# owensgroup/sparsify.me

Measured on AMD Instinct MI355X. Metric: effective GF/s (2:4 spmma vs dense gemm) on ResNet-50 layer shapes, higher is better.
Workload: dtype f16

## Files before the change

include/sparsifyme.h:

```cpp
#ifndef SPARSIFYME_H_
#define SPARSIFYME_H_

#include <stddef.h>
#include <stdint.h>

#ifdef __cplusplus
extern "C" {
#endif

#define SM_STATUS_SUCCESS 0
#define SM_STATUS_INVALID_VALUE 1
#define SM_STATUS_NOT_SUPPORTED 2
#define SM_STATUS_LAUNCH_FAILED 3
#define SM_STATUS_NO_DEVICE 4

#define SM_PRUNE_TILE 0
#define SM_PRUNE_STRIP 1

#define SM_OP_N 0
#define SM_OP_T 1

typedef void* sm_stream_t;

const char* sm_version(void);
// ... 78 lines not shown
int sm_prune24_spmma_f16(const void* A_in, void* A_out, const void* B, void* C, size_t m, size_t n, size_t k, size_t lda,
                         size_t batch, size_t strideA, size_t strideB, size_t strideC, int alg, int* d_valid, float alpha,
                         float beta, sm_stream_t stream);
int sm_prune24_spmma_bf16(const void* A_in, void* A_out, const void* B, void* C, size_t m, size_t n, size_t k, size_t lda,
                          size_t batch, size_t strideA, size_t strideB, size_t strideC, int alg, int* d_valid, float alpha,
                          float beta, sm_stream_t stream);

int sm_spmma_f16(const void* blob, const void* B, void* C, size_t m, size_t n, size_t k,
                 size_t batch, size_t strideB, size_t strideC, float alpha, float beta,
                 sm_stream_t stream);
int sm_spmma_f32(const void* blob, const float* B, float* C, size_t m, size_t n, size_t k,
                 size_t batch, size_t strideB, size_t strideC, float alpha, float beta,
                 sm_stream_t stream);

int sm_spmma_fused_f16(const void* A, const void* B, void* C, size_t m, size_t n, size_t k, size_t lda,
                       size_t batch, size_t strideA, size_t strideB, size_t strideC, float alpha,
                       float beta, sm_stream_t stream);

int sm_spmma_f16_grouped(size_t count, const void* const* blobs, const void* const* B, void* const* C, size_t m, size_t n, size_t k,
                         size_t batch, size_t strideB, size_t strideC, float alpha, float beta, sm_stream_t stream);
int sm_spmma_bf16_grouped(size_t count, const void* const* blobs, const void* const* B, void* const* C, size_t m, size_t n, size_t k,
                          size_t batch, size_t strideB, size_t strideC, float alpha, float beta, sm_stream_t stream);

int sm_spmma_fused_f16_grouped(size_t count, const void* const* A, const void* const* B, void* const* C, size_t m, size_t n,
                               size_t k, size_t lda, size_t batch, size_t strideA, size_t strideB, size_t strideC,
                               float alpha, float beta, sm_stream_t stream);
int sm_spmma_fused_bf16_grouped(size_t count, const void* const* A, const void* const* B, void* const* C, size_t m, size_t n,
                                size_t k, size_t lda, size_t batch, size_t strideA, size_t strideB, size_t strideC,
                                float alpha, float beta, sm_stream_t stream);

int sm_spmma_fused_workspace_size(size_t* bytes);
int sm_spmma_fused_workspace_state(const void* workspace, int* state, sm_stream_t stream);
int sm_spmma_fused_streamk_plan(size_t rows, size_t n, size_t k, size_t problems, int* takes, unsigned* plan);
#define SM_FUSED_FORM_NOT_TAKEN 0
#define SM_FUSED_FORM_EMPTY 1
#define SM_FUSED_FORM_THIN 2
#define SM_FUSED_FORM_SPAN 3
#define SM_FUSED_FORM_STREAMK 4
#define SM_FUSED_FORM_BIG 5
#define SM_FUSED_FORM_DIRECT64 6
#define SM_FUSED_FORM_DIRECT128 7
#define SM_FUSED_FORM_DIRECT128_NT 8
#define SM_FUSED_FORM_ASTAT 9
#define SM_FUSED_FORM_WIDEP 10
#define SM_FUSED_FORM_WIDE 11
#define SM_FUSED_FORM_WIDE_NT 12
#define SM_FUSED_FLAG_A_ALIGNED 1u
#define SM_FUSED_FLAG_B_ALIGNED 2u
#define SM_FUSED_FLAG_C_ALIGNED 4u
#define SM_FUSED_FLAG_WORKSPACE 8u
#define SM_FUSED_FLAG_EPILOGUE 16u
int sm_spmma_fused_form(size_t m, size_t n, size_t k, size_t lda, size_t batch, size_t count, size_t strideA, size_t strideB, size_t strideC,
                        float beta, unsigned flags, size_t cus, int* form);
int sm_gemm_rowmajor_f16_ws(const void* A, const void* B, void* C, size_t m, size_t n, size_t k, size_t lda, size_t batch, size_t strideA,
                            size_t strideB, size_t strideC, float alpha, float beta, void* workspace, size_t workspace_bytes, sm_stream_t stream);
int sm_gemm_rowmajor_bf16_ws(const void* A, const void* B, void* C, size_t m, size_t n, size_t k, size_t lda, size_t batch, size_t strideA,
                             size_t strideB, size_t strideC, float alpha, float beta, void* workspace, size_t workspace_bytes, sm_stream_t stream);
int sm_gemm_batched_f16_ws(const void* const* A_ptrs, const void* const* B_ptrs, void* const* C_ptrs, size_t m, size_t n, size_t k, size_t batch,
                           int transpose_a, int transpose_b, float alpha, float beta, void* workspace, size_t workspace_bytes, sm_stream_t stream);
int sm_spmma_fused_f16_ws(const void* A, const void* B, void* C, size_t m, size_t n, size_t k, size_t lda, size_t batch, size_t strideA,
                          size_t strideB, size_t strideC, float alpha, float beta, void* workspace, size_t workspace_bytes, sm_stream_t stream);
int sm_spmma_fused_bf16_ws(const void* A, const void* B, void* C, size_t m, size_t n, size_t k, size_t lda, size_t batch, size_t strideA,
                           size_t strideB, size_t strideC, float alpha, float beta, void* workspace, size_t workspace_bytes, sm_stream_t stream);
int sm_spmma_fused_f16_grouped_ws(size_t count, const void* const* A, const void* const* B, void* const* C, size_t m, size_t n,
                                  size_t k, size_t lda, size_t batch, size_t strideA, size_t strideB, size_t strideC,
                                  float alpha, float beta, void* workspace, size_t workspace_bytes, sm_stream_t stream);
int sm_spmma_fused_bf16_grouped_ws(size_t count, const void* const* A, const void* const* B, void* const* C, size_t m, size_t n,
                                   size_t k, size_t lda, size_t batch, size_t strideA, size_t strideB, size_t strideC,
                                   float alpha, float beta, void* workspace, size_t workspace_bytes, sm_stream_t stream);

#define SM_BIAS_COL 0
#define SM_BIAS_ROW 1
#define SM_ACT_NONE 0
#define SM_ACT_RELU 1
#define SM_ACT_CLIPPED_RELU 2
#define SM_ACT_LEAKY_RELU 3
#define SM_ACT_HARDSWISH 4
typedef struct {
  const float* bias;
  int bias_dim;
  int act;
  float act_arg;
  const void* R;
  size_t strideR;
} sm_epilogue_t;
int sm_spmma_f16_ex(const void* blob, const void* B, void* D, size_t m, size_t n, size_t k, size_t batch, size_t strideB,
                    size_t strideD, float alpha, float beta, const sm_epilogue_t* epilogue, sm_stream_t stream);
int sm_spmma_bf16_ex(const void* blob, const void* B, void* D, size_t m, size_t n, size_t k, size_t batch, size_t strideB,
                     size_t strideD, float alpha, float beta, const sm_epilogue_t* epilogue, sm_stream_t stream);
int sm_spmma_fused_f16_ex(const void* A, const void* B, void* D, size_t m, size_t n, size_t k, size_t lda, size_t batch,
                          size_t strideA, size_t strideB, size_t strideD, float alpha, float beta, const sm_epilogue_t* epilogue,
                          sm_stream_t stream);
int sm_spmma_fused_bf16_ex(const void* A, const void* B, void* D, size_t m, size_t n, size_t k, size_t lda, size_t batch,
                           size_t strideA, size_t strideB, size_t strideD, float alpha, float beta, const sm_epilogue_t* epilogue,
                           sm_stream_t stream);

int sm_linear24_f16(const void* blob, const void* X, void* Y, size_t tokens, size_t out_features, size_t in_features, size_t ldx,
                    size_t ldy, float alpha, float beta, const sm_epilogue_t* epilogue, sm_stream_t stream);
int sm_linear24_bf16(const void* blob, const void* X, void* Y, size_t tokens, size_t out_features, size_t in_features, size_t ldx,
                     size_t ldy, float alpha, float beta, const sm_epilogue_t* epilogue, sm_stream_t stream);

int sm_linear24_fp8(const void* blob, const void* X, void* Y, size_t tokens, size_t out_features, size_t in_features, size_t ldx,
                    size_t ldy, int fmt_w, int fmt_x, int out_type, float alpha, float beta, const float* w_scale, const float* x_scale,
                    const sm_epilogue_t* epilogue, sm_stream_t stream);
#define SM_LINEAR24_FORM_NOT_TAKEN 0
#define SM_LINEAR24_FORM_EMPTY 1
// ... 305 lines not shown
```

sparsify.me_amd/__init__.py:

```python
import ctypes
import os
import subprocess

_HERE = os.path.dirname(os.path.abspath(__file__))
LIB_PATH = os.environ.get("SPARSIFYME_LIB") or os.path.join(_HERE, "libsparsifyme.so")

PRUNE_TILE = 0
PRUNE_STRIP = 1
STATUS_SUCCESS, STATUS_INVALID_VALUE, STATUS_NOT_SUPPORTED, STATUS_LAUNCH_FAILED, STATUS_NO_DEVICE = 0, 1, 2, 3, 4

_lib = None

_c_size = ctypes.c_size_t
_c_ptr = ctypes.c_void_p
_c_f = ctypes.c_float
_c_i = ctypes.c_int

_SIGS = {
    "sm_device_check": [],
    "sm_sparsify_positional": [_c_ptr, _c_ptr, _c_size, _c_size, _c_size, _c_size, _c_size, _c_f, _c_ptr],
    "sm_sparsify_positional_f16": [_c_ptr, _c_ptr, _c_size, _c_size, _c_f, _c_ptr],
    "sm_sparsify_positional_f32": [_c_ptr, _c_ptr, _c_size, _c_size, _c_f, _c_ptr],
    "sm_sparsify_positional_f64": [_c_ptr, _c_ptr, _c_size, _c_size, _c_f, _c_ptr],
    "sm_prune24_f16": [_c_ptr, _c_ptr, _c_size, _c_size, _c_size, _c_i, _c_ptr],
# ... 43 lines not shown
                            _c_ptr],
    "sm_spmm_bell_batched_workspace_size": [_c_size, _c_size, _c_size, ctypes.POINTER(_c_size)],
    "sm_spmm_bell_batched_f32": [_c_ptr, _c_ptr, _c_size, _c_size, _c_size, _c_size, _c_ptr, _c_ptr, _c_size, _c_size, _c_f,
                                 _c_f, _c_ptr, _c_ptr],
    "sm_spmm_coo_workspace_size": [_c_size, ctypes.POINTER(_c_size)],
    "sm_spmm_coo_packed_workspace_size": [_c_size, _c_size, ctypes.POINTER(_c_size)],
    "sm_spmm_coo_f32_packed": [_c_size, _c_size, _c_size, _c_size, _c_size, _c_ptr, _c_ptr, _c_ptr, _c_ptr, _c_ptr, _c_f, _c_f,
                               _c_ptr, _c_size, _c_ptr],
    "sm_spmm_coo_f32_ws": [_c_size, _c_size, _c_size, _c_size, _c_size, _c_ptr, _c_ptr, _c_ptr, _c_ptr, _c_ptr, _c_f, _c_f,
                           _c_ptr, _c_ptr],
    "sm_spmm_coo_fast_workspace_size": [_c_size, _c_size, _c_size, _c_size, ctypes.POINTER(_c_size)],
    "sm_spmm_coo_fast_flag": [_c_ptr, ctypes.POINTER(_c_i), _c_ptr],
    "sm_spmm_coo_fast_form": [_c_size, _c_size, _c_size, _c_size, _c_size, _c_f],
    "sm_spmm_coo_f32_fast": [_c_size, _c_size, _c_size, _c_size, _c_size, _c_ptr, _c_ptr, _c_ptr, _c_ptr, _c_ptr, _c_f, _c_f,
                             _c_ptr, _c_size, _c_ptr],
    "sm_fill_uniform_f16": [_c_ptr, _c_size, ctypes.c_uint64, _c_f, _c_f, _c_ptr],
    "sm_fill_uniform_f32": [_c_ptr, _c_size, ctypes.c_uint64, _c_f, _c_f, _c_ptr],
    "sm_copy_bytes": [_c_ptr, _c_ptr, _c_size, _c_ptr],
}
_SIGS["sm_prune24_compress24_f16"] = [_c_ptr, _c_ptr, _c_size, _c_size, _c_size, _c_size, _c_size, _c_ptr, _c_ptr, _c_i, _c_ptr]
_SIGS["sm_prune24_compress24_bf16"] = _SIGS["sm_prune24_compress24_f16"]
_SIGS["sm_prune24_spmma_f16"] = [_c_ptr, _c_ptr, _c_ptr, _c_ptr] + [_c_size] * 8 + [_c_i, _c_ptr, _c_f, _c_f, _c_ptr]
_SIGS["sm_prune24_spmma_bf16"] = _SIGS["sm_prune24_spmma_f16"]
_SIGS["sm_prune24_compress24_f32"] = _SIGS["sm_prune24_compress24_f16"]
_SIGS["sm_prune24_form"] = [_c_ptr, _c_ptr, _c_size, _c_size, _c_size, _c_size, _c_i, ctypes.POINTER(_c_i), ctypes.POINTER(ctypes.c_uint)]
_SIGS["sm_prune24_check_form"] = [_c_ptr, _c_ptr, _c_size, _c_size, _c_size, _c_size, ctypes.POINTER(_c_i)]
_SIGS["sm_compress24_form"] = [_c_ptr, _c_ptr, _c_size, _c_size, _c_size, _c_size, _c_size, _c_size, ctypes.POINTER(_c_i)]
_SIGS["sm_decompress24_form"] = _SIGS["sm_compress24_form"]
_SIGS["sm_prune24_compress24_form"] = [_c_ptr, _c_ptr, _c_size, _c_size, _c_size, _c_size, _c_size, _c_ptr, _c_size, _c_i, _c_size,
                                       ctypes.POINTER(_c_i), ctypes.POINTER(ctypes.c_uint)]
_SIGS["sm_conv_spmma_fused_f16"] = [_c_ptr, _c_ptr, _c_ptr] + [_c_size] * 10 + [_c_f, _c_f, _c_ptr]
_SIGS["sm_conv_spmma_fused_bf16"] = _SIGS["sm_conv_spmma_fused_f16"]
_SIGS["sm_conv_spmma_fused_plan"] = [_c_size] * 10 + [ctypes.c_uint, ctypes.POINTER(_c_i), ctypes.POINTER(ctypes.c_uint)]
_SIGS["sm_transpose"] = [_c_ptr, _c_ptr] + [_c_size] * 8 + [_c_ptr]
_SIGS["sm_conv_out_size"] = [_c_size, _c_size, _c_size, _c_size, _c_size, ctypes.POINTER(_c_size)]
_SIGS["sm_im2col_f16"] = [_c_ptr] + [_c_size] * 9 + [_c_ptr, _c_ptr]
_SIGS["sm_im2col_compress24_f16"] = [_c_ptr] + [_c_size] * 9 + [_c_ptr, _c_ptr]
for _name in ("sm_prune24", "sm_prune24_check", "sm_compress24", "sm_decompress24"):
    _SIGS[_name + "_i8"] = _SIGS[_name + "_f16"]
_SIGS["sm_spmma_fused_i8"] = [_c_ptr, _c_ptr, _c_ptr] + [_c_size] * 8 + [_c_i, _c_ptr]
_SIGS["sm_spmma_fused_i8_q"] = [_c_ptr, _c_ptr, _c_ptr] + [_c_size] * 8 + [_c_f, _c_ptr]
_SIGS["sm_transpose_i8"] = [_c_ptr, _c_ptr, _c_size, _c_size, _c_ptr]
_SIGS["sm_spmma_i8"] = [_c_ptr, _c_ptr, _c_ptr, _c_size, _c_size, _c_size, _c_size, _c_size, _c_size, _c_i, _c_ptr]
_SIGS["sm_spmma_i8_q"] = [_c_ptr, _c_ptr, _c_ptr, _c_size, _c_size, _c_size, _c_size, _c_size, _c_size, _c_f, _c_ptr]
for _name in ("sm_prune24", "sm_prune24_check", "sm_compress24", "sm_decompress24", "sm_spmma", "sm_spmma_fused",
              "sm_gemm_rowmajor", "sm_fill_uniform", "sm_im2col", "sm_im2col_compress24"):
    _SIGS[_name + "_bf16"] = _SIGS[_name + "_f16"]
_SIGS["sm_spmma_fused_f32_split_prepare"] = [_c_ptr, _c_size, _c_size, _c_size, _c_size, _c_i, _c_ptr, _c_size, _c_ptr]
_SIGS["sm_spmma_fused_f32_split_prepared"] = [_c_ptr, _c_ptr, _c_ptr] + [_c_size] * 8 + [_c_i, _c_size, _c_f, _c_f, _c_ptr]
_SIGS["sm_spmma_fused_workspace_size"] = [ctypes.POINTER(_c_size)]
_SIGS["sm_spmma_fused_workspace_state"] = [_c_ptr, ctypes.POINTER(_c_i), _c_ptr]
_SIGS["sm_spmma_fused_streamk_plan"] = [_c_size, _c_size, _c_size, _c_size, ctypes.POINTER(_c_i), ctypes.POINTER(ctypes.c_uint)]
_SIGS["sm_spmma_fused_form"] = [_c_size] * 9 + [_c_f, ctypes.c_uint, _c_size, ctypes.POINTER(_c_i)]
_SIGS["sm_gemm_rowmajor_f16_ws"] = [_c_ptr, _c_ptr, _c_ptr] + [_c_size] * 8 + [_c_f, _c_f, _c_ptr, _c_size, _c_ptr]
_SIGS["sm_gemm_rowmajor_bf16_ws"] = _SIGS["sm_gemm_rowmajor_f16_ws"]
_SIGS["sm_gemm_batched_f16_ws"] = [_c_ptr, _c_ptr, _c_ptr, _c_size, _c_size, _c_size, _c_size, _c_i, _c_i, _c_f, _c_f, _c_ptr, _c_size, _c_ptr]
_SIGS["sm_spmma_fused_f16_ws"] = [_c_ptr, _c_ptr, _c_ptr] + [_c_size] * 8 + [_c_f, _c_f, _c_ptr, _c_size, _c_ptr]
_SIGS["sm_spmma_fused_bf16_ws"] = _SIGS["sm_spmma_fused_f16_ws"]
_SIGS["sm_spmma_fused_f16_grouped_ws"] = [_c_size, _c_ptr, _c_ptr, _c_ptr] + [_c_size] * 8 + [_c_f, _c_f, _c_ptr, _c_size, _c_ptr]
_SIGS["sm_spmma_fused_bf16_grouped_ws"] = _SIGS["sm_spmma_fused_f16_grouped_ws"]
_SIGS["sm_spmm_bell_f16"] = _SIGS["sm_spmm_bell_f32"]
_SIGS["sm_spmm_bell_bf16"] = _SIGS["sm_spmm_bell_f32"]
_SIGS["sm_spmm_bell_batched_f16"] = [_c_ptr, _c_ptr, _c_size, _c_size, _c_size, _c_size, _c_ptr, _c_ptr, _c_size, _c_size, _c_f, _c_f, _c_ptr]
_SIGS["sm_spmm_bell_batched_bf16"] = _SIGS["sm_spmm_bell_batched_f16"]
_SIGS["sm_prune24_fp8"] = [_c_ptr, _c_ptr, _c_size, _c_size, _c_size, _c_i, _c_i, _c_ptr]
_SIGS["sm_prune24_check_fp8"] = _SIGS["sm_prune24_check_f16"]
_SIGS["sm_compress24_fp8"] = [_c_ptr, _c_size, _c_size, _c_size, _c_size, _c_size, _c_ptr, _c_i, _c_ptr]
_SIGS["sm_decompress24_fp8"] = _SIGS["sm_decompress24_f16"]
_SIGS["sm_spmma_fp8"] = [_c_ptr, _c_ptr, _c_ptr] + [_c_size] * 6 + [_c_i, _c_i, _c_i, _c_f, _c_f, _c_ptr, _c_ptr]
_SIGS["sm_spmma_fused_fp8"] = [_c_ptr, _c_ptr, _c_ptr] + [_c_size] * 8 + [_c_i, _c_i, _c_i, _c_f, _c_f, _c_ptr, _c_ptr]
_SIGS["sm_gemm_rowmajor_fp8"] = _SIGS["sm_spmma_fused_fp8"]
_SIGS["sm_gemm_rowmajor_i8"] = _SIGS["sm_spmma_fused_i8"]
_SIGS["sm_gemm_rowmajor_i8_q"] = _SIGS["sm_spmma_fused_i8_q"]
for _sfx16 in ("f16", "bf16"):
    _SIGS["sm_quantize_rows_fp8_" + _sfx16] = [_c_ptr, _c_size, _c_size, _c_size, _c_ptr, _c_size, _c_ptr, _c_i, _c_ptr]
    _SIGS["sm_quantize_compress24_fp8_" + _sfx16] = [_c_ptr, _c_size, _c_size, _c_size, _c_ptr, _c_ptr, _c_i, _c_ptr]
    _SIGS["sm_quantize_transpose_fp8_" + _sfx16] = [_c_ptr, _c_size, _c_size, _c_size, _c_f, _c_ptr, _c_i, _c_ptr]
for _sfx16 in ("f16", "bf16"):
    _SIGS["sm_spmma_%s_ex" % _sfx16] = _SIGS["sm_spmma_f16"][:-1] + [_c_ptr, _c_ptr]
    _SIGS["sm_spmma_fused_%s_ex" % _sfx16] = _SIGS["sm_spmma_fused_f16"][:-1] + [_c_ptr, _c_ptr]
for _sfx16 in ("f16", "bf16"):
    _SIGS["sm_linear24_" + _sfx16] = [_c_ptr, _c_ptr, _c_ptr] + [_c_size] * 5 + [_c_f, _c_f, _c_ptr, _c_ptr]
_SIGS["sm_linear24_fp8"] = [_c_ptr, _c_ptr, _c_ptr] + [_c_size] * 5 + [_c_i, _c_i, _c_i, _c_f, _c_f, _c_ptr, _c_ptr, _c_ptr, _c_ptr]
_SIGS["sm_linear24_fp8_form"] = [_c_size] * 4 + [ctypes.POINTER(_c_i)]
for _sfx16 in ("f16", "bf16"):
    _SIGS["sm_linear24_glu_" + _sfx16] = [_c_ptr, _c_ptr, _c_ptr] + [_c_size] * 5 + [_c_i, _c_ptr, _c_ptr]
_SIGS["sm_linear24_glu_fp8"] = [_c_ptr, _c_ptr, _c_ptr] + [_c_size] * 5 + [_c_i, _c_i, _c_i, _c_i, _c_ptr, _c_ptr, _c_ptr, _c_ptr]
_SIGS["sm_linear24_glu_form"] = [_c_size] * 4 + [ctypes.POINTER(_c_i)]
for _sfx16 in ("f16", "bf16", "fp8"):
    _SIGS["sm_linear24_grouped_" + _sfx16] = _SIGS["sm_linear24_" + _sfx16][:3] + [_c_ptr, _c_size] + _SIGS["sm_linear24_" + _sfx16][3:]
    _SIGS["sm_linear24_grouped_glu_" + _sfx16] = _SIGS["sm_linear24_glu_" + _sfx16][:3] + [_c_ptr, _c_size] + _SIGS["sm_linear24_glu_" + _sfx16][3:]
_SIGS["sm_linear24_grouped_form"] = [_c_size] * 5 + [ctypes.POINTER(_c_i)]
for _sfx16 in ("f16", "bf16", "fp8"):
    for _g in ("sm_linear24_grouped_", "sm_linear24_grouped_glu_"):
        _SIGS[_g + "gather_" + _sfx16] = _SIGS[_g + _sfx16][:4] + [_c_ptr, _c_size] + _SIGS[_g + _sfx16][4:]
_SIGS["sm_moe_route_workspace_size"] = [_c_size] * 3 + [ctypes.POINTER(_c_size)]
_SIGS["sm_moe_route"] = [_c_ptr] + [_c_size] * 3 + [_c_ptr] * 5 + [_c_size, _c_ptr]
_SIGS["sm_moe_route_form"] = [_c_size] * 3 + [ctypes.POINTER(_c_i)]
for _sfx16 in ("f16", "bf16"):
    _SIGS["sm_moe_combine_" + _sfx16] = [_c_ptr] * 5 + [_c_size] * 6 + [_c_ptr]
_SIGS["sm_moe_combine_form"] = [_c_ptr] * 3 + [_c_size] * 3 + [ctypes.POINTER(_c_i)]
for _sfx3 in ("f16", "bf16", "f32"):
    _SIGS["sm_moe_gate_" + _sfx3] = [_c_ptr] * 4 + [_c_size] * 4 + [_c_i, _c_i, _c_f, _c_ptr]
_SIGS["sm_moe_gate_form"] = [_c_size] * 3 + [ctypes.POINTER(_c_i)]
for _sfx16 in ("f16", "bf16"):
    _SIGS["sm_rmsnorm_" + _sfx16] = [_c_ptr] * 7 + [_c_size] * 6 + [_c_f, _c_i, _c_ptr]
# ... 698 lines not shown


def gemm_rowmajor_i8(A, B, C, m, n, k, lda=None, batch=1, strideA=None, strideB=0, strideC=None, accumulate=False):
    lda = k if lda is None else lda
    strideA = m * lda if strideA is None else strideA
    strideC = m * n if strideC is None else strideC
    if C.dtype != _t().int32:
        raise SparsifymeError("gemm_rowmajor_i8 writes int32; use gemm_rowmajor_i8_q for a requantised int8 result")
    _check(lib().sm_gemm_rowmajor_i8(_dev(A), _dev(B), _dev(C), m, n, k, lda, batch, strideA, strideB, strideC, 1 if accumulate else 0,
                                     _stream()), "sm_gemm_rowmajor_i8")


def gemm_rowmajor_i8_q(A, B, C, m, n, k, scale, lda=None, batch=1, strideA=None, strideB=0, strideC=None):
    lda = k if lda is None else lda
    strideA = m * lda if strideA is None else strideA
    strideC = m * n if strideC is None else strideC
    if C.dtype != _t().int8:
        raise SparsifymeError("gemm_rowmajor_i8_q writes int8")
    _check(lib().sm_gemm_rowmajor_i8_q(_dev(A), _dev(B), _dev(C), m, n, k, lda, batch, strideA, strideB, strideC, float(scale), _stream()),
           "sm_gemm_rowmajor_i8_q")


def spmma_fused_workspace_size():
    out = _c_size(0)
    _check(lib().sm_spmma_fused_workspace_size(ctypes.byref(out)), "sm_spmma_fused_workspace_size")
    return out.value


def spmma_fused_streamk_plan(rows, n, k, problems=1):
    takes = _c_i(0)
    buf = (ctypes.c_uint * 32)()
    _check(lib().sm_spmma_fused_streamk_plan(rows, n, k, problems, ctypes.byref(takes), buf), "sm_spmma_fused_streamk_plan")
    v = list(buf)
    return bool(takes.value), dict(tg=v[0], wg=v[1], groups_full=v[2], tgl=v[3], wgl=v[4], slots=v[5], units=v[6], cut=v[7:16], cutl=v[16:25])


FUSED_FORMS = ("not_taken", "empty", "thin", "span", "streamk", "big", "direct64", "direct128", "direct128_nt", "astat", "widep", "wide", "wide_nt")
FUSED_FLAG_A_ALIGNED, FUSED_FLAG_B_ALIGNED, FUSED_FLAG_C_ALIGNED, FUSED_FLAG_WORKSPACE, FUSED_FLAG_EPILOGUE = 1, 2, 4, 8, 16


def spmma_fused_form(m, n, k, lda=None, batch=1, count=1, strideA=None, strideB=0, strideC=None, beta=0.0, a_aligned=True, b_aligned=True,
                     c_aligned=True, workspace=False, epilogue=False, cus=0):
    lda = k if lda is None else lda
    strideA = m * lda if strideA is None else strideA
    strideC = m * n if strideC is None else strideC
    flags = ((FUSED_FLAG_A_ALIGNED if a_aligned else 0) | (FUSED_FLAG_B_ALIGNED if b_aligned else 0) | (FUSED_FLAG_C_ALIGNED if c_aligned else 0) |
             (FUSED_FLAG_WORKSPACE if workspace else 0) | (FUSED_FLAG_EPILOGUE if epilogue else 0))
    form = _c_i(-1)
    _check(lib().sm_spmma_fused_form(m, n, k, lda, batch, count, strideA, strideB, strideC, float(beta), flags, cus, ctypes.byref(form)),
           "sm_spmma_fused_form")
    return FUSED_FORMS[form.value]


def streamk_whole_panels(plan, panels, nkt):
    cuts = set()
    for g in range(plan["groups_full"]):
        cuts.update(g * plan["tg"] * nkt + c for c in plan["cut"][:plan["wg"] + 1])
    base = plan["groups_full"] * plan["tg"] * nkt
    cuts.update(base + c for c in plan["cutl"][:plan["wgl"] + 1])
    return [t for t in range(panels) if not any(t * nkt < u < (t + 1) * nkt for u in cuts)]


def spmma_fused_workspace_state(ws):
    st = _c_i(-1)
    _check(lib().sm_spmma_fused_workspace_state(_dev(ws), ctypes.byref(st), _stream()), "sm_spmma_fused_workspace_state")
    return st.value


def spmma_fused_workspace():
    return _t().zeros(spmma_fused_workspace_size(), dtype=_t().uint8, device="cuda")


def spmma_fused(A, B, C, m, n, k, lda=None, batch=1, strideA=None, strideB=0, strideC=None, alpha=1.0, beta=0.0, workspace=None,
                epilogue=None):
    lda = k if lda is None else lda
    strideA = m * lda if strideA is None else strideA
    strideC = m * n if strideC is None else strideC
    if epilogue is not None:
        if workspace is not None:
            raise SparsifymeError("spmma_fused: the workspace (stream-K) form takes no epilogue")
        st = epilogue.struct_for(C, strideC, float(beta))
        fn = getattr(lib(), "sm_spmma_fused_%s_ex" % _sfx(A))
        _check(fn(_dev(A), _dev(B), _dev(C), m, n, k, lda, batch, strideA, strideB, strideC, float(alpha), float(beta), ctypes.addressof(st),
                  _stream()), "sm_spmma_fused_ex")
        return
    if workspace is not None:
        fn = getattr(lib(), "sm_spmma_fused_%s_ws" % _sfx(A))
        _check(fn(_dev(A), _dev(B), _dev(C), m, n, k, lda, batch, strideA, strideB, strideC, float(alpha), float(beta), _dev(workspace),
                  workspace.numel() * workspace.element_size(), _stream()), "sm_spmma_fused_ws")
        return
    fn = getattr(lib(), "sm_spmma_fused_" + _sfx(A))
    _check(fn(_dev(A), _dev(B), _dev(C), m, n, k, lda, batch, strideA, strideB, strideC, float(alpha), float(beta), _stream()),
           "sm_spmma_fused")


def spmma_grouped(blobs, Bs, Cs, m, n, k, batch=1, strideB=0, strideC=None, alpha=1.0, beta=0.0):
    if not (len(blobs) == len(Bs) == len(Cs)):
        raise SparsifymeError("spmma_grouped: operand lists differ in length")
    if not blobs:
        return
    if strideC is None:
        strideC = m * n
    fn = getattr(lib(), "sm_spmma_%s_grouped" % _sfx(Bs[0]))
    _check(fn(len(blobs), _ptr_table(blobs), _ptr_table(Bs), _ptr_table(Cs), m, n, k, batch, strideB, strideC, float(alpha), float(beta),
              _stream()), "sm_spmma_grouped")

# ... 190 lines not shown
```

sparsify.me_amd/csrc/spmma_f16_fused.hip:

```cpp
#include "select24.h"
#include "spmma_args.h"

namespace sm {

constexpr int MAXG = 8;
struct FusedArgs {
  const half_t* A[MAXG];
  const half_t* B[MAXG];
  half_t* C[MAXG];
  size_t sA, sB, sC;
  int Mrows, N, K, lda;
  int batch, tiles_m, tiles_n;
  int ngroup;
  float alpha, beta;
  const half_t* const* dAp;
  const half_t* const* dBp;
  half_t* const* dCp;
};

struct FusedArgsEpi : FusedArgs {
  EpiArgs e;
};
template <bool EPI> struct FusedArgsSel { typedef FusedArgs type; };
template <> struct FusedArgsSel<true> { typedef FusedArgsEpi type; };
// ... 482 lines not shown
  const SkPlan pl = sk_plan(panels, nkt, tn, cus);
  const size_t nwg = (size_t)pl.slots * tn;
  if (pl.slots == 0 || nwg > cus || nwg > 1023) return "sm_spmma_fused_*_ws: the shape has more column tiles than the stream-K form has compute units for";
  return nullptr;
}

template <int BN, bool BF = false, bool ANT = true, bool DENSE = false>
static int launch_fused_sk(const FusedArgs& a0, void* workspace, size_t workspace_bytes, hipStream_t st) {
  constexpr int BM = 256;
  static_assert(BN == 256, "sk_launch_limits counts 256-column tiles");
  FusedArgs a = a0;
  a.tiles_m = (a.Mrows + BM - 1) / BM;
  a.tiles_n = (a.N + BN - 1) / BN;
  const size_t panels = (size_t)a.tiles_m * a.batch * a.ngroup;
  if (panels == 0) return SM_STATUS_SUCCESS;
  const size_t nkt = (size_t)a.K / 64;
  const int cus = device_cu_count();
  if (const char* why = sk_launch_limits(panels, (size_t)a.N, (size_t)a.K, (size_t)a.lda, (size_t)cus)) {
    set_error("%s", why);
    return SM_STATUS_NOT_SUPPORTED;
  }
  SkPlan pl = sk_plan(panels, nkt, (size_t)a.tiles_n, (size_t)cus);
  const size_t nwg = (size_t)pl.slots * a.tiles_n;
  if (!workspace || !aligned16(workspace) || workspace_bytes < sk_workspace_bytes(nwg, BN)) {
    set_error("sm_spmma_fused_*_ws: the stream-K form needs a 16-byte aligned workspace of sm_spmma_fused_workspace_size bytes");
    return SM_STATUS_INVALID_VALUE;
  }
  SkArgs s = {};
  s.flags = reinterpret_cast<unsigned*>(workspace);
  s.part = reinterpret_cast<float*>(reinterpret_cast<char*>(workspace) + 4096);
  s.panels = (unsigned)panels; s.slots = pl.slots; s.tg = pl.tg; s.wg = pl.wg; s.groups_full = pl.groups_full; s.tgl = pl.tgl; s.wgl = pl.wgl;
  for (int i = 0; i < 9; ++i) { s.cut[i] = pl.cut[i]; s.cutl[i] = pl.cutl[i]; }
  constexpr size_t lds_main = (size_t)3 * BM * 128 + (size_t)2 * 64 * BN * 2;
  constexpr size_t lds_epi = (size_t)BM * (BN * 2 + 16);
  constexpr size_t lds = lds_main > lds_epi ? lds_main : lds_epi;
  static_assert(lds > 64 * 1024 && lds <= 160 * 1024, "LDS budget of the stream-K kernel (always opted in)");
  return launch_grid<&spmma_f16_fused_sk_kernel<BN, BF, ANT, DENSE>>(nwg, 512, lds, lds, st, "sm_spmma_fused_f16", "spmma_f16_fused_sk_kernel", a, s);
}

static bool sk_takes(size_t rows, size_t problems, size_t n, size_t k, bool astat_shape, size_t cus, SkPlan& pl) {
  if (n <= 128 || k < 128 || k % 64 != 0) return false;
  const size_t nkt = k / 64;
  const size_t panels = (rows + 255) / 256 * problems, tn = (n + 255) / 256;
  const size_t t_big = panels * tn, t_wide = (rows + 127) / 128 * tn * problems;
  pl = sk_plan(panels, nkt, tn, cus);
  if (!pl.slots) return false;
  const double c_sk = (double)pl.units + (pl.wg > 1 ? 8.0 : 0.0);
  const double c_big = (double)((t_big + cus - 1) / cus * nkt), c_wide = 0.6 * (double)((t_wide + cus - 1) / cus * nkt);
  const double c_now = c_big < c_wide ? c_big : c_wide;
  return !astat_shape && pl.wg > 1 && c_sk < 0.85 * c_now;
}

__device__ __attribute__((aligned(256))) const unsigned char sm_fused_zero_page[256] = {0};

template <int BN, bool BF = false, bool DENSE = false, bool EPI = false>
__global__ __launch_bounds__(256) void spmma_f16_fused_span_kernel(const typename FusedArgsSel<EPI>::type p, const unsigned span_lds ,
                                                                   const size_t a_bytes ) {
  constexpr int BM = 128, NW = 4, TM = BM / NW, FM = TM / 16, FN = BN / 16;
  constexpr int SB = 64 * BN * 2;
  extern __shared__ __attribute__((aligned(16))) char smem[];
  const unsigned tid = threadIdx.x, lane = tid & 63u;
  const unsigned wave = __builtin_amdgcn_readfirstlane(tid >> 6);
  const unsigned tiles = (unsigned)p.tiles_m * (unsigned)p.tiles_n;
  const unsigned lid = xcd_remap(blockIdx.x, gridDim.x);
  const unsigned grp = lid / tiles, trem = lid - grp * tiles;
  const unsigned tile_m = trem / (unsigned)p.tiles_n, tile_n = trem - tile_m * (unsigned)p.tiles_n;
  const int m0 = (int)tile_m * BM, n0 = (int)tile_n * BN;
  const int nkt = (p.K + 63) / 64;
  const char* A = reinterpret_cast<const char*>(p.dAp ? p.dAp[grp] : p.A[grp]);
  const half_t* B = p.dBp ? p.dBp[grp] : p.B[grp];
  half_t* C = p.dCp ? p.dCp[grp] : p.C[grp];
  const unsigned rowbytes = (unsigned)p.K * 2u;
  const int rows = p.Mrows - m0 < BM ? p.Mrows - m0 : BM;
  EpiBias<FM, FN> eb;
  if constexpr (EPI) eb = epi_bias_prefetch<FM, FN>(p.e, true, wave * TM, 0, m0, n0, p.Mrows, p.N, lane);

  {
    const size_t s0 = (size_t)m0 * rowbytes;
    const unsigned len = (unsigned)rows * rowbytes;
    const unsigned np = (len + 1023u) / 1024u;
    const size_t last16 = a_bytes - 16;
    for (unsigned pc = wave; pc < np; pc += NW) {
      size_t off = s0 + (size_t)pc * 1024u + 16u * lane;
      off = off < last16 ? off : last16;
      __builtin_amdgcn_global_load_lds((gptr_t*)(A + off), (lptr_t*)(smem + pc * 1024u), 16, 0, 2);
    }
  }
  char* const Bimg = smem + span_lds;
  {
    constexpr int B_N = BN / 8;
    const int npb = nkt * B_N;
    for (int t = (int)wave; t < npb; t += NW) {
      const int kt = t / B_N, j = t - kt * B_N;
      const unsigned panel = (unsigned)j >> 3, kr = 8u * ((unsigned)j & 7u) + (lane >> 3);
      const unsigned cs = (lane & 7u) ^ b_swz(kr);
      int gc = n0 + (int)(64u * panel + 8u * cs);
      gc = gc <= p.N - 8 ? gc : p.N - 8;
      const int krow = kt * 64 + (int)kr;
      const char* src = krow < p.K ? reinterpret_cast<const char*>(B + (size_t)krow * p.N + gc)
                                   : reinterpret_cast<const char*>(sm_fused_zero_page) + 16u * (lane & 7u);
      __builtin_amdgcn_global_load_lds((gptr_t*)src, (lptr_t*)(Bimg + kt * SB + panel * 8192u + ((unsigned)j & 7u) * 1024u), 16, 0, 0);
    }
  }
  wait_dma_and_barrier<0>();

  f4 acc[FM][FN];
#pragma unroll
  for (int i = 0; i < FM; ++i)
#pragma unroll
    for (int j = 0; j < FN; ++j) acc[i][j] = f4{0.f, 0.f, 0.f, 0.f};
  const unsigned g = lane >> 4, r = lane & 15u;
  unsigned rowoff[FM];
#pragma unroll
  for (int i = 0; i < FM; ++i) {
    int row = (int)(wave * TM + i * 16 + r);
    row = row < rows ? row : rows - 1;
    rowoff[i] = (unsigned)row * rowbytes;
  }
  for (int kt = 0; kt < nkt; ++kt) {
    if constexpr (DENSE) {
      h8 a0[FM], a1[FM];
#pragma unroll
      for (int i = 0; i < FM; ++i) {
        uint32_t d[2][4];
#pragma unroll
        for (int h = 0; h < 2; ++h) {
          const int k0 = kt * 64 + 32 * h + 8 * (int)g;
          int nv = p.K - k0;
          nv = nv < 0 ? 0 : (nv > 8 ? 8 : nv);
          const char* src = smem + rowoff[i] + 2u * (unsigned)k0;
#pragma unroll
          for (int e = 0; e < 4; ++e) {
            const uint32_t lo16 = *reinterpret_cast<const unsigned short*>(src + 4 * e);
            const uint32_t hi16 = *reinterpret_cast<const unsigned short*>(src + 4 * e + 2);
            uint32_t v = lo16 | (hi16 << 16);
            v = 2 * e + 1 < nv ? v : (2 * e < nv ? (v & 0xffffu) : 0u);
            d[h][e] = v;
          }
        }
        a0[i] = __builtin_bit_cast(h8, u4{d[0][0], d[0][1], d[0][2], d[0][3]});
        a1[i] = __builtin_bit_cast(h8, u4{d[1][0], d[1][1], d[1][2], d[1][3]});
      }
      mfma_b_sweep<FM, FN, BF>(a0, a1, Bimg + kt * SB, 0, lane, acc);
      continue;
    }
    h8 af[FM];
    int idx[FM];
    const int k0 = kt * 64 + 16 * (int)g;
    int nv = p.K - k0;
    nv = nv < 0 ? 0 : (nv > 16 ? 16 : nv);
#pragma unroll
    for (int i = 0; i < FM; ++i) {
      const char* src = smem + rowoff[i] + 2u * (unsigned)k0;
      uint32_t d[8];
#pragma unroll
      for (int e = 0; e < 8; ++e) {
        const uint32_t lo16 = *reinterpret_cast<const unsigned short*>(src + 4 * e);
        const uint32_t hi16 = *reinterpret_cast<const unsigned short*>(src + 4 * e + 2);
        uint32_t v = lo16 | (hi16 << 16);
        v = 2 * e + 1 < nv ? v : (2 * e < nv ? (v & 0xffffu) : 0u);
        d[e] = v;
      }
      dense16_to_operand(u4{d[0], d[1], d[2], d[3]}, u4{d[4], d[5], d[6], d[7]}, af[i], idx[i]);
    }
    smfmac_b_sweep<FM, FN, BF>(af, idx, Bimg + kt * SB, 0, lane, acc);
  }
  __syncthreads();
  if constexpr (EPI) store_c_tile_epi<BM, BN, FM, FN, 64 * NW, BF>(smem, C, p.e.R, p.e, eb, acc, true, wave * TM, 0, m0, n0, p.Mrows, p.N, p.alpha, p.beta, tid);
  else store_c_tile<BM, BN, FM, FN, 64 * NW, BF>(smem, C, acc, true, wave * TM, 0, m0, n0, p.Mrows, p.N, p.alpha, p.beta, tid);
}

template <int BN, bool BF = false, bool DENSE = false, bool EPI = false>
static int launch_fused_span(const typename FusedArgsSel<EPI>::type& a0, hipStream_t st) {
  typename FusedArgsSel<EPI>::type a = a0;
  a.tiles_m = (a.Mrows + 127) / 128;
  a.tiles_n = (a.N + BN - 1) / BN;
  const size_t nwg = (size_t)a.tiles_m * a.tiles_n * a.ngroup;
  if (nwg == 0) return SM_STATUS_SUCCESS;
  const size_t kc = ((size_t)a.K + 63) / 64 * 64;
  const size_t span_lds = ((size_t)128 * a.K * 2 + 128 + 1023) / 1024 * 1024;
  const size_t lds_main = span_lds + kc * BN * 2;
  constexpr size_t lds_epi = (size_t)128 * (BN * 2 + 16);
  const size_t lds = lds_main > lds_epi ? lds_main : lds_epi;
  if (lds > 160 * 1024 || nwg > 0x7fffffffu) {
    set_error("sm_spmma_fused_{f16,bf16}: k too long for the span form (use the staged path)");
    return SM_STATUS_NOT_SUPPORTED;
  }
  return launch_grid<&spmma_f16_fused_span_kernel<BN, BF, DENSE, EPI>>(nwg, 256, 160 * 1024, lds, st, "sm_spmma_fused_f16", "spmma_f16_fused_span_kernel", a,
                                                                      (unsigned)span_lds, (size_t)a.Mrows * a.K * 2);
}

template <int BN, int NBW>
struct BTileDma {
  static constexpr int B_WI = (BN / 8) / NBW;
  const char* src[B_WI];
  unsigned dst[B_WI];
  size_t step;
  __device__ __forceinline__ void setup(const half_t* B, int N, int n0, unsigned bw, unsigned lane, unsigned ring_off) {
#pragma unroll
    for (int i = 0; i < B_WI; ++i) {
      const unsigned j = bw + (unsigned)NBW * i, panel = j >> 3, grp = j & 7u, kr = 8u * grp + (lane >> 3);
      const unsigned cs = (lane & 7u) ^ b_swz(kr);
      int gc = n0 + (int)(64u * panel + 8u * cs);
      gc = gc <= N - 8 ? gc : N - 8;
      src[i] = reinterpret_cast<const char*>(B) + ((size_t)kr * N + (size_t)gc) * 2;
      dst[i] = ring_off + panel * 8192u + grp * 1024u;
    }
    step = (size_t)64 * N * 2;
  }
  __device__ __forceinline__ void issue(char* smem, int kt, unsigned buf_off) const {
#pragma unroll
    for (int i = 0; i < B_WI; ++i)
      __builtin_amdgcn_global_load_lds((gptr_t*)(src[i] + (size_t)kt * step), (lptr_t*)(smem + buf_off + dst[i]), 16, 0, 0);
  }
};


template <int BN, int WM, int WN, int NLB, int PF, int NSB, bool BF = false, bool ANT = true, bool EPI = false>
__global__ __launch_bounds__(64 * (WM * WN + 4 + NLB)) void spmma_f16_fused_wide_kernel(const typename FusedArgsSel<EPI>::type p) {
  constexpr int BM = 128, NLA = 4, NC = WM * WN, NW = NC + NLA + NLB;
  static_assert(PF >= 1 && PF <= 3 && NSB >= 2 && NSB <= 4, "pipeline depths");
  constexpr int TM = BM / WM, TN = BN / WN, FM = TM / 16, FN = TN / 16;
  constexpr int SA = BM * 64, SM_ = BM * 8, ASTG = SA + SM_, SB = 64 * BN * 2;
  constexpr int BRING = 2 * ASTG;
  constexpr int NBW = NLB > 0 ? NLB : WM * WN;
  constexpr int B_N = BN / 8, B_WI = B_N / NBW;
  static_assert(B_N % NBW == 0 && B_WI >= 1 && (NSB - 2) * B_WI <= 63, "B tile vs issuing waves");
  extern __shared__ __attribute__((aligned(16))) char smem[];

  const unsigned tid = threadIdx.x, lane = tid & 63u;
  const unsigned wave = __builtin_amdgcn_readfirstlane(tid >> 6);
// ... 701 lines not shown
    return {SM_FUSED_FORM_NOT_TAKEN, false, "sm_spmma_fused_{f16,bf16}_grouped: needs 16-byte aligned C operands"};
  if (!dims_fit_int(m, n, k, lda, batch)) return {SM_FUSED_FORM_NOT_TAKEN, false, "sm_spmma_fused_{f16,bf16}: dimension exceeds 2^31-1"};
  const bool stacked = batch > 1 && contiguous && (!c.epi || c.beta == 0.0f || c.sR == m * n);
  const size_t rows = stacked ? m * batch : m, nb = (stacked ? 1 : batch) * c.count;
  const bool astat_store = n > 256 && k <= 512 && c.beta == 0.0f && c.c_aligned && (c.sC % 8 == 0);
  if (c.ws) {
    SkPlan pl;
    if (sk_takes(rows, nb, n, k, astat_store, cus, pl) && c.ws_bytes >= sk_workspace_bytes((size_t)pl.slots * ((n + 255) / 256), 256) && c.ws_aligned &&
        !sk_launch_limits((rows + 255) / 256 * nb, n, k, lda, cus))
      return {SM_FUSED_FORM_STREAMK, stacked, nullptr};
  }
  auto round_eff = [](size_t tiles, size_t cus_) { const size_t r = (tiles + cus_ - 1) / cus_; return r ? (double)tiles / (double)(r * cus_) : 1.0; };
  if (n > 128 && k > 64) {
    const size_t t_big = (rows + 255) / 256 * ((n + 255) / 256) * nb, t_wide = (rows + 127) / 128 * ((n + 255) / 256) * nb;
    bool big = round_eff(t_big, cus) >= round_eff(t_wide, cus);
    if (!c.epi && astat_store) {
      const size_t panels = (rows + 127) / 128 * nb;
      big = round_eff(t_big, cus) > round_eff(panels * astat_nsplit(panels, (n + 127) / 128, cus), cus) + 0.1;
    }
    if (big) return {SM_FUSED_FORM_BIG, stacked, nullptr};
  }
  if (n <= 128 || (n <= 256 && k <= 64)) {
    if (n <= 64) return {SM_FUSED_FORM_DIRECT64, stacked, nullptr};
    return {n > 128 || k < 512 ? SM_FUSED_FORM_DIRECT128 : SM_FUSED_FORM_DIRECT128_NT, stacked, nullptr};
  }
  if (!c.epi && astat_store && astat_lds_bytes((int)(k / 64), 3) <= 160 * 1024) return {SM_FUSED_FORM_ASTAT, stacked, nullptr};
  if (k <= 1024 && !c.epi) return {SM_FUSED_FORM_WIDEP, stacked, nullptr};
  return {n > 256 ? SM_FUSED_FORM_WIDE : SM_FUSED_FORM_WIDE_NT, stacked, nullptr};
}

static bool fused_form_is_exact(int form) { return form != SM_FUSED_FORM_NOT_TAKEN && form != SM_FUSED_FORM_EMPTY && form != SM_FUSED_FORM_THIN; }

bool sm::spmma_fused16_takes_exact(const void* A, const void* B, const void* C, size_t m, size_t n, size_t k, size_t lda, size_t batch, size_t strideA, size_t strideB,
                                   size_t strideC) {
  if (!A || !B || !C || lda < k) return false;
  const FusedCall c = {m, n, k, lda, batch, 1, strideA, strideB, strideC, 0.0f, aligned16(A), aligned16(B), aligned16(C), false, false, 0, false, false, 0};
  return fused_form_is_exact(fused_form(c, 256).form);
}

extern "C" int sm_spmma_fused_form(size_t m, size_t n, size_t k, size_t lda, size_t batch, size_t count, size_t strideA, size_t strideB, size_t strideC,
                                   float beta, unsigned flags, size_t cus, int* form) {
  constexpr unsigned known = SM_FUSED_FLAG_A_ALIGNED | SM_FUSED_FLAG_B_ALIGNED | SM_FUSED_FLAG_C_ALIGNED | SM_FUSED_FLAG_WORKSPACE | SM_FUSED_FLAG_EPILOGUE;
  if (!form || lda < k || count > (size_t)MAXG || (flags & ~known) || ((flags & SM_FUSED_FLAG_WORKSPACE) && (flags & SM_FUSED_FLAG_EPILOGUE))) {
    set_error("sm_spmma_fused_form: invalid argument");
    return SM_STATUS_INVALID_VALUE;
  }
  const bool c_al = (flags & SM_FUSED_FLAG_C_ALIGNED) != 0, ws = (flags & SM_FUSED_FLAG_WORKSPACE) != 0;
  const FusedCall c = {m, n, k, lda, batch, count, strideA, strideB, strideC, beta, (flags & SM_FUSED_FLAG_A_ALIGNED) != 0, (flags & SM_FUSED_FLAG_B_ALIGNED) != 0, c_al,
                       ws, ws, ws ? ~(size_t)0 : 0, (flags & SM_FUSED_FLAG_EPILOGUE) != 0, c_al, strideC};
  *form = fused_form(c, cus ? cus : (size_t)device_cu_count()).form;
  return SM_STATUS_SUCCESS;
}

template <bool BF>
static int spmma_fused16(size_t ngroup, const void* const* Ag, const void* const* Bg, void* const* Cg, size_t m, size_t n, size_t k, size_t lda,
                         size_t batch, size_t strideA, size_t strideB, size_t strideC, float alpha, float beta,
                         sm_stream_t stream, void* workspace = nullptr, size_t workspace_bytes = 0, const EpiArgs* epi = nullptr) {
#define SM_LAUNCH(fn, ...) (epi ? fn<__VA_ARGS__, true>(ae, st) : fn<__VA_ARGS__, false>(a, st))
  if (ngroup == 0) return SM_STATUS_SUCCESS;
  if (!Ag || !Bg || !Cg || lda < k || ngroup > (size_t)MAXG) {
    set_error("sm_spmma_fused_{f16,bf16}: invalid argument");
    return SM_STATUS_INVALID_VALUE;
  }
  FusedCall c = {m, n, k, lda, batch, ngroup, strideA, strideB, strideC, beta, true, true, true, workspace != nullptr, aligned16(workspace), workspace_bytes,
                 epi != nullptr, epi && aligned16(epi->R), epi ? epi->sR : 0};
  for (size_t g = 0; g < ngroup; ++g) {
    if (!Ag[g] || !Bg[g] || !Cg[g]) {
      set_error("sm_spmma_fused_{f16,bf16}: invalid argument (null operand)");
      return SM_STATUS_INVALID_VALUE;
    }
    c.a_aligned = c.a_aligned && aligned16(Ag[g]);
    c.b_aligned = c.b_aligned && aligned16(Bg[g]);
    c.c_aligned = c.c_aligned && aligned16(Cg[g]);
  }
  const FusedPick pick = fused_form(c, (size_t)device_cu_count());
  hipStream_t st = (hipStream_t)stream;
  FusedArgs a = {};
  for (size_t g = 0; g < (size_t)MAXG; ++g) {
    const size_t s_ = g < ngroup ? g : 0;
    a.A[g] = (const half_t*)Ag[s_]; a.B[g] = (const half_t*)Bg[s_]; a.C[g] = (half_t*)Cg[s_];
  }
  a.ngroup = (int)ngroup;
  a.N = (int)n; a.K = (int)k; a.lda = (int)lda;
  a.alpha = alpha; a.beta = beta;
  if (pick.stacked) {
    a.Mrows = (int)(m * batch);
    a.batch = 1;
  } else {
    a.Mrows = (int)m;
    a.batch = (int)batch;
  }
  if (pick.form != SM_FUSED_FORM_SPAN) { a.sA = strideA; a.sB = strideB; a.sC = strideC; }
  FusedArgsEpi ae = {};
  static_cast<FusedArgs&>(ae) = a;
  if (epi) ae.e = *epi;
  switch (pick.form) {
    case SM_FUSED_FORM_EMPTY: return SM_STATUS_SUCCESS;
    case SM_FUSED_FORM_NOT_TAKEN:
      set_error("%s", pick.why);
      return SM_STATUS_NOT_SUPPORTED;
    case SM_FUSED_FORM_THIN: return spmma_fused_thin(BF, (int)ngroup, Ag, Bg, Cg, m * batch, n, k, alpha, beta, st);
    case SM_FUSED_FORM_SPAN: return n <= 64 ? SM_LAUNCH(launch_fused_span, 64, BF, false) : SM_LAUNCH(launch_fused_span, 128, BF, false);
    case SM_FUSED_FORM_STREAMK:
      return n <= 256 ? launch_fused_sk<256, BF, true>(a, workspace, workspace_bytes, st) : launch_fused_sk<256, BF, false>(a, workspace, workspace_bytes, st);
    case SM_FUSED_FORM_BIG: return n <= 256 ? SM_LAUNCH(launch_fused_big, 256, BF, 3, 2, true, false) : SM_LAUNCH(launch_fused_big, 256, BF, 3, 2, false, false);
    case SM_FUSED_FORM_DIRECT64: return SM_LAUNCH(launch_fused_direct, 64, 2, BF, 128, 4, true, false);
// ... 158 lines not shown
```

Measured before the change: 570,100.

## Add double-buffered ring kernel for ragged-K span form of fused 2:4 spmma

Result: no change. 573,400, median of 6 (+0.6%).

```diff
diff --git a/include/sparsifyme.h b/include/sparsifyme.h
--- a/include/sparsifyme.h
+++ b/include/sparsifyme.h
@@ -154,6 +154,10 @@
 #define SM_FUSED_FLAG_EPILOGUE 16u
 int sm_spmma_fused_form(size_t m, size_t n, size_t k, size_t lda, size_t batch, size_t count, size_t strideA, size_t strideB, size_t strideC,
                         float beta, unsigned flags, size_t cus, int* form);
+#define SM_FUSED_SPAN_KERNEL_NONE 0
+#define SM_FUSED_SPAN_KERNEL_ONESHOT 1
+#define SM_FUSED_SPAN_KERNEL_RING 2
+int sm_spmma_fused_span_kernel(size_t m, size_t n, size_t k, size_t batch, size_t count, unsigned flags, int* which);
 int sm_gemm_rowmajor_f16_ws(const void* A, const void* B, void* C, size_t m, size_t n, size_t k, size_t lda, size_t batch, size_t strideA,
                             size_t strideB, size_t strideC, float alpha, float beta, void* workspace, size_t workspace_bytes, sm_stream_t stream);
 int sm_gemm_rowmajor_bf16_ws(const void* A, const void* B, void* C, size_t m, size_t n, size_t k, size_t lda, size_t batch, size_t strideA,
diff --git a/sparsify.me_amd/__init__.py b/sparsify.me_amd/__init__.py
--- a/sparsify.me_amd/__init__.py
+++ b/sparsify.me_amd/__init__.py
@@ -119,6 +119,7 @@
 _SIGS["sm_spmma_fused_workspace_state"] = [_c_ptr, ctypes.POINTER(_c_i), _c_ptr]
 _SIGS["sm_spmma_fused_streamk_plan"] = [_c_size, _c_size, _c_size, _c_size, ctypes.POINTER(_c_i), ctypes.POINTER(ctypes.c_uint)]
 _SIGS["sm_spmma_fused_form"] = [_c_size] * 9 + [_c_f, ctypes.c_uint, _c_size, ctypes.POINTER(_c_i)]
+_SIGS["sm_spmma_fused_span_kernel"] = [_c_size] * 5 + [ctypes.c_uint, ctypes.POINTER(_c_i)]
 _SIGS["sm_gemm_rowmajor_f16_ws"] = [_c_ptr, _c_ptr, _c_ptr] + [_c_size] * 8 + [_c_f, _c_f, _c_ptr, _c_size, _c_ptr]
 _SIGS["sm_gemm_rowmajor_bf16_ws"] = _SIGS["sm_gemm_rowmajor_f16_ws"]
 _SIGS["sm_gemm_batched_f16_ws"] = [_c_ptr, _c_ptr, _c_ptr, _c_size, _c_size, _c_size, _c_size, _c_i, _c_i, _c_f, _c_f, _c_ptr, _c_size, _c_ptr]
@@ -923,6 +924,17 @@
     return FUSED_FORMS[form.value]
 
 
+FUSED_SPAN_KERNELS = ("none", "oneshot", "ring")
+
+
+def spmma_fused_span_kernel(m, n, k, batch=1, count=1, a_aligned=True, b_aligned=True, c_aligned=True, epilogue=False):
+    flags = ((FUSED_FLAG_A_ALIGNED if a_aligned else 0) | (FUSED_FLAG_B_ALIGNED if b_aligned else 0) | (FUSED_FLAG_C_ALIGNED if c_aligned else 0) |
+             (FUSED_FLAG_EPILOGUE if epilogue else 0))
+    which = _c_i(-1)
+    _check(lib().sm_spmma_fused_span_kernel(m, n, k, batch, count, flags, ctypes.byref(which)), "sm_spmma_fused_span_kernel")
+    return FUSED_SPAN_KERNELS[which.value]
+
+
 def streamk_whole_panels(plan, panels, nkt):
     cuts = set()
     for g in range(plan["groups_full"]):
diff --git a/sparsify.me_amd/csrc/spmma_f16_fused.hip b/sparsify.me_amd/csrc/spmma_f16_fused.hip
--- a/sparsify.me_amd/csrc/spmma_f16_fused.hip
+++ b/sparsify.me_amd/csrc/spmma_f16_fused.hip
@@ -558,6 +558,19 @@
 }
 
 __device__ __attribute__((aligned(256))) const unsigned char sm_fused_zero_page[256] = {0};
+
+template <bool MASK>
+__device__ __forceinline__ void ragged_row_to_operand(const char* As, const unsigned (&foff)[9], unsigned sh, int nv, h8& af, int& idx) {
+  uint32_t w[9], d[8];
+#pragma unroll
+  for (int e = 0; e < 9; ++e) w[e] = *reinterpret_cast<const uint32_t*>(As + foff[e]);
+#pragma unroll
+  for (int e = 0; e < 8; ++e) {
+    d[e] = __builtin_amdgcn_alignbit(w[e + 1], w[e], sh);
+    if constexpr (MASK) d[e] = 2 * e + 1 < nv ? d[e] : (2 * e < nv ? (d[e] & 0xffffu) : 0u);
+  }
+  dense16_to_operand(u4{d[0], d[1], d[2], d[3]}, u4{d[4], d[5], d[6], d[7]}, af, idx);
+}
 
 template <int BN, bool BF = false, bool DENSE = false, bool EPI = false>
 __global__ __launch_bounds__(256) void spmma_f16_fused_span_kernel(const typename FusedArgsSel<EPI>::type p, const unsigned span_lds ,
@@ -657,23 +670,154 @@
     nv = nv < 0 ? 0 : (nv > 16 ? 16 : nv);
 #pragma unroll
     for (int i = 0; i < FM; ++i) {
-      const char* src = smem + rowoff[i] + 2u * (unsigned)k0;
-      uint32_t d[8];
-#pragma unroll
-      for (int e = 0; e < 8; ++e) {
-        const uint32_t lo16 = *reinterpret_cast<const unsigned short*>(src + 4 * e);
-        const uint32_t hi16 = *reinterpret_cast<const unsigned short*>(src + 4 * e + 2);
-        uint32_t v = lo16 | (hi16 << 16);
-        v = 2 * e + 1 < nv ? v : (2 * e < nv ? (v & 0xffffu) : 0u);
-        d[e] = v;
-      }
-      dense16_to_operand(u4{d[0], d[1], d[2], d[3]}, u4{d[4], d[5], d[6], d[7]}, af[i], idx[i]);
+      const unsigned addr = rowoff[i] + 2u * (unsigned)k0;
+      unsigned fo[9];
+#pragma unroll
+      for (int e = 0; e < 9; ++e) fo[e] = (addr & ~3u) + 4u * (unsigned)e;
+      if (kt + 1 == nkt) ragged_row_to_operand<true>(smem, fo, 8u * (addr & 2u), nv, af[i], idx[i]);
+      else ragged_row_to_operand<false>(smem, fo, 8u * (addr & 2u), 16, af[i], idx[i]);
     }
     smfmac_b_sweep<FM, FN, BF>(af, idx, Bimg + kt * SB, 0, lane, acc);
   }
   __syncthreads();
   if constexpr (EPI) store_c_tile_epi<BM, BN, FM, FN, 64 * NW, BF>(smem, C, p.e.R, p.e, eb, acc, true, wave * TM, 0, m0, n0, p.Mrows, p.N, p.alpha, p.beta, tid);
   else store_c_tile<BM, BN, FM, FN, 64 * NW, BF>(smem, C, acc, true, wave * TM, 0, m0, n0, p.Mrows, p.N, p.alpha, p.beta, tid);
+}
+
+template <int BN, bool BF = false>
+__global__ __launch_bounds__(256) void spmma_f16_fused_ragged_ring_kernel(const FusedArgs p) {
+  constexpr int BM = 128, NW = 4, TM = BM / NW, FM = TM / 16, FN = BN / 16, NS = 2;
+  constexpr int SA = BM * 128, ST = BM * 16, SB = 64 * BN * 2, STAGE = SA + ST + SB;
+  constexpr int A_N = BM / 8, T_N = ST / 1024, B_N = BN / 8, SLA = A_N / NW, SLB = B_N / NW;
+  static_assert(A_N % NW == 0 && B_N % NW == 0 && T_N == 2, "DMA pieces per wave");
+  static_assert(BN == 64 || BN == 128, "column tile");
+  static_assert(NS * STAGE == (BN == 64 ? 52 : 68) * 1024, "a stage: 16 KiB + 2 KiB of A, 8 or 16 KiB of B; a ring of two");
+  static_assert(BN == 64 ? 3 * NS * STAGE <= 160 * 1024 : (2 * NS * STAGE <= 160 * 1024 && 3 * NS * STAGE > 160 * 1024),
+                "workgroups per CU: three at 64 columns, two at 128");
+  static_assert(BM * (BN * 2 + 16) <= STAGE, "the C tile's transposition fits one stage");
+  extern __shared__ __attribute__((aligned(16))) char smem[];
+  const unsigned tid = threadIdx.x, lane = tid & 63u;
+  const unsigned wave = __builtin_amdgcn_readfirstlane(tid >> 6);
+  const unsigned tiles = (unsigned)p.tiles_m * (unsigned)p.tiles_n;
+  const unsigned lid = tile_order(blockIdx.x, gridDim.x, true);
+  const unsigned grp = lid / tiles, trem = lid - grp * tiles;
+  const unsigned tile_m = trem / (unsigned)p.tiles_n, tile_n = trem - tile_m * (unsigned)p.tiles_n;
+  const int m0 = (int)tile_m * BM, n0 = (int)tile_n * BN;
+  const int nkt = (p.K + 63) / 64;
+  const unsigned rowbytes = (unsigned)p.K * 2u;
+  const int rows = p.Mrows - m0 < BM ? p.Mrows - m0 : BM;
+  const size_t s0 = (size_t)m0 * rowbytes;
+  const char* const At = reinterpret_cast<const char*>(p.A[grp]) + s0;
+  const char* const B = reinterpret_cast<const char*>(p.B[grp]);
+  half_t* C = p.C[grp];
+
+  unsigned asrc[SLA], aend[SLA], tsrc, tend, bsrc[SLB];
+#pragma unroll
+  for (int i = 0; i < SLA; ++i) {
+    const unsigned t = wave + (unsigned)NW * i;
+    const unsigned row = 8u * t + (lane >> 3), cs = (lane & 7u) ^ (row & 7u);
+    const unsigned rr = (int)row < rows ? row : (unsigned)(rows - 1);
+    asrc[i] = ((rr * rowbytes) & ~15u) + 16u * cs;
+    aend[i] = (rr * rowbytes + rowbytes - 2u) & ~15u;
+  }
+  {
+    const unsigned row = 64u * (wave & 1u) + lane;
+    const unsigned rr = (int)row < rows ? row : (unsigned)(rows - 1);
+    tsrc = ((rr * rowbytes) & ~15u) + 128u;
+    tend = (rr * rowbytes + rowbytes - 2u) & ~15u;
+  }
+  unsigned bkr[SLB];
+#pragma unroll
+  for (int i = 0; i < SLB; ++i) {
+    const unsigned j = wave + (unsigned)NW * i, panel = j >> 3, kr = 8u * (j & 7u) + (lane >> 3);
+    const unsigned cs = (lane & 7u) ^ b_swz(kr);
+    int gc = n0 + (int)(64u * panel + 8u * cs);
+    gc = gc <= p.N - 8 ? gc : p.N - 8;
+    bsrc[i] = (kr * (unsigned)p.N + (unsigned)gc) * 2u;
+    bkr[i] = kr;
+  }
+  const unsigned bstep = 64u * (unsigned)p.N * 2u;
+  const char* const zero = reinterpret_cast<const char*>(sm_fused_zero_page) + 16u * (lane & 7u);
+  auto stage = [&](int kt, int buf) {
+    char* base = smem + buf * STAGE;
+    const unsigned ka = 128u * (unsigned)kt;
+#pragma unroll
+    for (int i = 0; i < SLA; ++i) {
+      unsigned off = asrc[i] + ka;
+      off = off < aend[i] ? off : aend[i];
+      __builtin_amdgcn_global_load_lds((gptr_t*)(At + off), (lptr_t*)(base + (wave + (unsigned)NW * i) * 1024u), 16, 0, 0);
+    }
+    if (wave < (unsigned)T_N) {
+      unsigned off = tsrc + ka;
+      off = off < tend ? off : tend;
+      __builtin_amdgcn_global_load_lds((gptr_t*)(At + off), (lptr_t*)(base + SA + wave * 1024u), 16, 0, 0);
+    }
+#pragma unroll
+    for (int i = 0; i < SLB; ++i) {
+      const unsigned j = wave + (unsigned)NW * i;
+      const char* src = kt * 64 + (int)bkr[i] < p.K ? B + ((size_t)kt * bstep + bsrc[i]) : zero;
+      __builtin_amdgcn_global_load_lds((gptr_t*)src, (lptr_t*)(base + SA + ST + (j >> 3) * 8192u + (j & 7u) * 1024u), 16, 0, 0);
+    }
+  };
+
+  const unsigned g = lane >> 4, r = lane & 15u;
+  unsigned foff[FM][9], sh;
+  {
+    const unsigned o = ((wave * TM + r) * rowbytes) & 15u;
+    sh = 8u * (o & 2u);
+#pragma unroll
+    for (int i = 0; i < FM; ++i) {
+      const unsigned row = wave * TM + i * 16 + r;
+#pragma unroll
+      for (int e = 0; e < 9; ++e) {
+        const unsigned w = (o >> 2) + 8u * g + (unsigned)e, c = w >> 2, j = w & 3u;
+        foff[i][e] = c < 8u ? a_off(row, c) + 4u * j : (unsigned)SA + row * 16u + 4u * j;
+      }
+    }
+  }
+
+  f4 acc[FM][FN];
+#pragma unroll
+  for (int i = 0; i < FM; ++i)
+#pragma unroll
+    for (int j = 0; j < FN; ++j) acc[i][j] = f4{0.f, 0.f, 0.f, 0.f};
+
+  stage(0, 0);
+  int cur = 0;
+  for (int kt = 0; kt + 1 < nkt; ++kt) {
+    wait_dma_and_barrier<0>();
+    stage(kt + 1, cur ^ 1);
+    const char* As = smem + cur * STAGE;
+    h8 af[FM];
+    int idx[FM];
+#pragma unroll
+    for (int i = 0; i < FM; ++i) ragged_row_to_operand<false>(As, foff[i], sh, 16, af[i], idx[i]);
+    smfmac_b_sweep<FM, FN, BF>(af, idx, As + SA + ST, 0, lane, acc);
+    cur ^= 1;
+  }
+  {
+    wait_dma_and_barrier<0>();
+    const char* As = smem + cur * STAGE;
+    int nv = p.K - ((nkt - 1) * 64 + 16 * (int)g);
+    nv = nv < 0 ? 0 : (nv > 16 ? 16 : nv);
+    h8 af[FM];
+    int idx[FM];
+#pragma unroll
+    for (int i = 0; i < FM; ++i) ragged_row_to_operand<true>(As, foff[i], sh, nv, af[i], idx[i]);
+    smfmac_b_sweep<FM, FN, BF>(af, idx, As + SA + ST, 0, lane, acc);
+  }
+  __syncthreads();
+  store_c_tile<BM, BN, FM, FN, 64 * NW, BF>(smem, C, acc, true, wave * TM, 0, m0, n0, p.Mrows, p.N, p.alpha, p.beta, tid);
+}
+
+static bool span_ring_takes(bool epi, bool dense, bool c_aligned) { return !epi && !dense && c_aligned; }
+
+template <int BN, bool BF = false>
+static int launch_fused_ragged_ring(const FusedArgs& a, hipStream_t st) {
+  const size_t nwg = (size_t)a.tiles_m * a.tiles_n * a.ngroup;
+  constexpr size_t stage_bytes = 128 * 128 + 128 * 16 + 64 * BN * 2;
+  const size_t lds = (a.K <= 64 ? 1 : 2) * stage_bytes;
+  return launch_grid<&spmma_f16_fused_ragged_ring_kernel<BN, BF>>(nwg, 256, 2 * stage_bytes, lds, st, "sm_spmma_fused_f16", "spmma_f16_fused_ragged_ring_kernel", a);
 }
 
 template <int BN, bool BF = false, bool DENSE = false, bool EPI = false>
@@ -683,6 +827,11 @@
   a.tiles_n = (a.N + BN - 1) / BN;
   const size_t nwg = (size_t)a.tiles_m * a.tiles_n * a.ngroup;
   if (nwg == 0) return SM_STATUS_SUCCESS;
+  if constexpr (!DENSE && !EPI) {
+    bool c_aligned = true;
+    for (int g = 0; g < a.ngroup; ++g) c_aligned = c_aligned && aligned16(a.C[g]);
+    if (span_ring_takes(EPI, DENSE, c_aligned) && nwg <= 0x7fffffffu) return launch_fused_ragged_ring<BN, BF>(a, st);
+  }
   const size_t kc = ((size_t)a.K + 63) / 64 * 64;
   const size_t span_lds = ((size_t)128 * a.K * 2 + 128 + 1023) / 1024 * 1024;
   const size_t lds_main = span_lds + kc * BN * 2;
@@ -1490,6 +1639,20 @@
   return SM_STATUS_SUCCESS;
 }
 
+extern "C" int sm_spmma_fused_span_kernel(size_t m, size_t n, size_t k, size_t batch, size_t count, unsigned flags, int* which) {
+  constexpr unsigned known = SM_FUSED_FLAG_A_ALIGNED | SM_FUSED_FLAG_B_ALIGNED | SM_FUSED_FLAG_C_ALIGNED | SM_FUSED_FLAG_EPILOGUE;
+  if (!which || count > (size_t)MAXG || (flags & ~known)) {
+    set_error("sm_spmma_fused_span_kernel: invalid argument");
+    return SM_STATUS_INVALID_VALUE;
+  }
+  const bool c_al = (flags & SM_FUSED_FLAG_C_ALIGNED) != 0, epi = (flags & SM_FUSED_FLAG_EPILOGUE) != 0;
+  const FusedCall c = {m, n, k, k, batch, count, m * k, 0, m * n, 0.0f, (flags & SM_FUSED_FLAG_A_ALIGNED) != 0, (flags & SM_FUSED_FLAG_B_ALIGNED) != 0, c_al,
+                       false, false, 0, epi, c_al, m * n};
+  if (fused_form(c, 256).form != SM_FUSED_FORM_SPAN) *which = SM_FUSED_SPAN_KERNEL_NONE;
+  else *which = span_ring_takes(epi, false, c_al) ? SM_FUSED_SPAN_KERNEL_RING : SM_FUSED_SPAN_KERNEL_ONESHOT;
+  return SM_STATUS_SUCCESS;
+}
+
 template <bool BF>
 static int spmma_fused16(size_t ngroup, const void* const* Ag, const void* const* Bg, void* const* Cg, size_t m, size_t n, size_t k, size_t lda,
                          size_t batch, size_t strideA, size_t strideB, size_t strideC, float alpha, float beta,
```
